# Pixel-Talk/CanonSwap

Hardware: AMD Instinct MI355X
Metric: frames/sec at 512x512 (generator hot path F->W->T->R->W->G) (higher is better)
Workload: dtype f16; 1 GPU; BASELINE configs[2]: 512x512 video, 64 frames batched per launch on each GPU, steady state over 1280 frames (20 launches per GPU) (256x256 crops in, random-init weights of the real architecture); frames_per_launch_per_gpu=64, frames_total=1280, parallelism=frame-shard x1, identities_resident=1, latency_mode=False, accumulate=fp32, debug_decodes=False

## Files before the change

canonswap_amd/_isa.py:

```python
from __future__ import annotations

import os
import subprocess

from ._build import HALO_NGROUPS, OBJ_DIR


def _disassemble(obj_dir: str, objdump: str, oname: str) -> str:
    obj = os.path.join(obj_dir, oname)
    subprocess.run([objdump, "--offloading", obj], check=True, capture_output=True)
    co = obj + ".0.hipv4-amdgcn-amd-amdhsa--gfx950"
    try:
        return subprocess.run([objdump, "-d", "--no-show-raw-insn", co], check=True, capture_output=True, text=True).stdout
    finally:
        for f in os.listdir(obj_dir):
            if f.startswith(oname + ".0."):
                os.remove(os.path.join(obj_dir, f))


def isa_check(obj_dir: str | None = None) -> dict:
    import re
    obj_dir = obj_dir or OBJ_DIR
    objdump = os.environ.get("LLVM_OBJDUMP", "/opt/rocm/lib/llvm/bin/llvm-objdump")
    if not os.path.exists(objdump):
        raise FileNotFoundError(f"isa_check: {objdump} not found")
    seen = dict(_isa_check_wide(obj_dir, objdump))
    seen.update(_isa_check_lat(obj_dir, objdump))
    for g in range(HALO_NGROUPS):
        txt = _disassemble(obj_dir, objdump, f"conv_halo_g{g}.o")
        for m in re.finditer(r"^[0-9a-f]+ <(_Z16conv_halo_kernelILi\d+ELi\d+ELi(\d+)ELi\d+ELi\d+ELi\d+ELb[01]ELb[01]ELi0EEv10ConvParams)>:\n(.*?)(?=^[0-9a-f]+ <|\Z)",
                             txt, re.S | re.M):
            name, wch, body = m.group(1), int(m.group(2)), m.group(3).split("\n")
            want = f"s_waitcnt vmcnt({3 * wch})"
            kend = max(i for i, l in enumerate(body) if "v_mfma" in l)
            waits = [i for i, l in enumerate(body) if i < kend and l.strip().startswith(want) and "lgkmcnt" not in l]
            if len(waits) < 4:
                raise RuntimeError(f"isa_check: {name}: {len(waits)} x `{want}` in the K loop, expected 4 (one per ring slot)")
            waits = waits[:4]
            loads = [(i, re.search(r"global_load_dwordx4 v\[(\d+):(\d+)\], v\[\d+:\d+\], off", l)) for i, l in enumerate(body)]
            loads = [(i, int(q.group(1))) for i, q in loads if q]
            prime = [r for i, r in loads if i < waits[0]][-4 * wch:]
            if len(prime) != 4 * wch:
                raise RuntimeError(f"isa_check: {name}: the prologue primes {len(prime)} ring registers, expected {4 * wch}")
            for k, w in enumerate(waits):
                slot = prime[k * wch:(k + 1) * wch]
                end = waits[k + 1] if k + 1 < 4 else len(body)
                seg = body[w:end]
                rel = [i for i, r in loads if w < i < end and r in slot]
                if len(rel) < wch:
                    raise RuntimeError(f"isa_check: {name}: ring slot {k} is not reloaded into v{slot} after its wait")
                first_reload = min(rel) - w
                uses = [j for j, l in enumerate(seg[:first_reload]) if "v_mfma" in l and any(f"v[{r}:{r + 3}]" in l for r in slot)]
                if not uses:
                    raise RuntimeError(f"isa_check: {name}: no MFMA reads ring slot {k} (v{slot}) between its wait and its reload")
            tail = "\n".join(body[waits[-1]:])
            if "s_waitcnt vmcnt(0)" not in tail:
                raise RuntimeError(f"isa_check: {name}: the ring is not drained (s_waitcnt vmcnt(0)) before the epilogue")
            seen[name] = len(waits)
    if not seen:
        raise RuntimeError("isa_check: no dynamic-shape conv_halo kernel found in the objects (name mangling changed?)")
    return seen


def _isa_check_lat(obj_dir: str, objdump: str) -> dict:
    import re
    txt = _disassemble(obj_dir, objdump, "conv_lat.o")
    seen = {}
    for m in re.finditer(r"^[0-9a-f]+ <(\S*conv_lat_kernel\S*)>:\n(.*?)(?=^[0-9a-f]+ <|\Z)", txt, re.S | re.M):
        name, body = m.group(1), [l.split("//")[0].strip() for l in m.group(2).split("\n")]
        body = [l for l in body if l]
        mf = [i for i, l in enumerate(body) if l.startswith("v_mfma")]
        if not mf:
            raise RuntimeError(f"isa_check: {name}: no MFMA")
        if any(l.startswith(("s_cbranch", "s_branch")) for l in body[mf[0]:mf[-1]]):
            raise RuntimeError(f"isa_check: {name}: a branch inside the K loop (the walk assumes straight-line code)")
        for i, l in enumerate(body):
            if re.search(r"\bm0\b", l):
                ok = l.startswith("s_mov_b32 m0,") and any(b.startswith("buffer_load") and b.endswith("lds") for b in body[i + 1:i + 3])
                if not ok:
                    raise RuntimeError(f"isa_check: {name}: `{l}` touches m0 outside the hidden LDS-DMA sequence")
        nvm, open_dma, nbar, ndma = 0, [], 0, 0
        for i, l in enumerate(body[:mf[-1] + 1]):
            op = l.split()[0]
            if op.startswith(("global_load", "buffer_load", "global_store", "buffer_store", "scratch_load", "scratch_store")):
                if op.startswith("buffer_load") and l.endswith("lds"):
                    open_dma.append(nvm); ndma += 1
                nvm += 1
            if op == "s_barrier":
                nbar += 1
                w = next((body[j] for j in range(i - 1, max(i - 6, -1), -1) if body[j].startswith("s_waitcnt") and "vmcnt" in body[j]), None)
                if w is None and not open_dma:
                    continue
                if w is None:
                    raise RuntimeError(f"isa_check: {name}: barrier {nbar} of the K loop has no vmcnt wait in front of it")
                n = int(re.search(r"vmcnt\((\d+)\)", w).group(1))
                for idx in open_dma:
                    if nvm - idx - 1 < n:
                        raise RuntimeError(f"isa_check: {name}: `{w}` before barrier {nbar} does not cover a DMA piece issued {nvm - idx - 1} vector-memory instructions earlier")
                open_dma = []
        if open_dma:
            raise RuntimeError(f"isa_check: {name}: {len(open_dma)} DMA pieces are never waited for at a chunk head")
        if len(mf) not in (8 * 6 * 8, 8 * 6 * 16) or ndma != 24:
            raise RuntimeError(f"isa_check: {name}: {len(mf)} MFMAs / {ndma} DMA instructions, expected 384 or 768 / 24")
        seen[name] = len(mf)
    if not seen:
        raise RuntimeError("isa_check: no conv_lat kernel found in conv_lat.o (name mangling changed?)")
    return seen


def _isa_check_wide(obj_dir: str, objdump: str) -> dict:
    seen = _isa_check_ring(obj_dir, objdump, "conv_wide.o", r"\S*conv_wide_kernel\S*", 18 * 64)
    seen.update(_isa_check_ring(obj_dir, objdump, "conv_halo_g1.o", r"_Z16conv_halo_kernelILi32ELi8ELi5ELi2ELi2ELi0ELb1ELb0ELi[789]E\S*", None))
    return seen


def _isa_check_ring(obj_dir: str, objdump: str, oname: str, name_re: str, expect_mfma) -> dict:
    import re
    txt = _disassemble(obj_dir, objdump, oname)
    seen = {}
    for m in re.finditer(r"^[0-9a-f]+ <(" + name_re + r")>:\n(.*?)(?=^[0-9a-f]+ <|\Z)", txt, re.S | re.M):
        name, body = m.group(1), m.group(2).split("\n")
        writer, waited, issued, nmfma = {}, {}, {}, 0
        pending, nvm = [], 0
        mf = [i for i, l in enumerate(body) if "v_mfma" in l]
        lo, hi = (mf[0], mf[-1]) if mf else (0, 0)
        for li, l in enumerate(body):
            t = l.split("//")[0].strip()
            if not t:
                continue
            op = t.split()[0]
            if op.startswith("s_waitcnt") and "vmcnt" in t:
                n = int(re.search(r"vmcnt\((\d+)\)", t).group(1))
                for r in waited:
                    if nvm - issued.get(r, -1) - 1 >= n:
                        waited[r] = True
                pending = [q for q in pending if nvm - q[1] - 1 < n]
            if op.startswith(("s_cbranch", "s_branch", "s_endpgm")) or li < lo:
                pending = []
            if pending and not op.startswith(("s_", "global_store", "buffer_store", "ds_write", "scratch_store")):
                mm0 = re.match(r"\S+\s+(v\[(\d+):(\d+)\]|v(\d+))", t)
                if mm0 and not (op.startswith("buffer_load") and t.endswith("lds")):
                    dst = set(range(int(mm0.group(2)), int(mm0.group(3)) + 1)) if mm0.group(2) else {int(mm0.group(4))}
                    for regs, _ in pending:
                        if regs & dst:
                            raise RuntimeError(f"isa_check: {name}: `{t}` writes v{sorted(regs & dst)} while an untracked ring load into them is in flight")
            if op.startswith(("global_load", "buffer_load", "global_store", "buffer_store", "scratch_load", "scratch_store", "global_atomic")):
                if op.startswith("global_load_dwordx4") and li >= lo:
                    q = re.match(r"\S+\s+v\[(\d+):(\d+)\]", t)
                    if q:
                        pending.append((set(range(int(q.group(1)), int(q.group(2)) + 1)), nvm))
                nvm += 1
            if op.startswith("v_mfma"):
                ops = re.findall(r"([av])\[(\d+):(\d+)\]", t)
                if len(ops) < 4 or ops[1][0] != "v":
                    raise RuntimeError(f"isa_check: {name}: MFMA with a weight operand outside the VGPRs: {t}")
                nmfma += 1
                for r in range(int(ops[1][1]), int(ops[1][2]) + 1):
                    if not writer.get(r, "").startswith("global_load_dwordx4"):
                        raise RuntimeError(f"isa_check: {name}: v{r}, a weight operand of `{t}`, was last written by `{writer.get(r)}` (a copy of a ring register?)")
                    if not waited.get(r, False):
                        raise RuntimeError(f"isa_check: {name}: no vmcnt wait between the ring load of v{r} and `{t}`")
                continue
            if op.startswith(("global_store", "buffer_store", "ds_write", "scratch_store", "s_", "buffer_load_dwordx4")) and "lds" in t + " lds" and not op.startswith("global_load"):
                if not op.startswith(("v_", "ds_read", "global_load", "scratch_load")):
                    continue
            mm = re.match(r"\S+\s+(v\[(\d+):(\d+)\]|v(\d+))", t)
            if mm and not op.startswith(("global_store", "buffer_store", "ds_write", "scratch_store")) and not (op.startswith("buffer_load") and t.endswith("lds")):
                rng = range(int(mm.group(2)), int(mm.group(3)) + 1) if mm.group(2) else [int(mm.group(4))]
                is_vm = op.startswith(("global_load", "buffer_load", "scratch_load"))
                for r in rng:
                    writer[r] = op
                    waited[r] = False
                    issued[r] = (nvm - 1) if is_vm else -1
        if expect_mfma is not None and nmfma != expect_mfma:
            raise RuntimeError(f"isa_check: {name}: {nmfma} MFMAs in the kernel, expected {expect_mfma}")
        seen[name] = nmfma
    if not seen:
        raise RuntimeError(f"isa_check: no kernel matching {name_re} found in {oname} (name mangling changed?)")
    return seen
```

canonswap_amd/csrc/vol32.hip:

```cpp
#include "conv_epilogue.h"

namespace {

constexpr int V_TW = 8;
constexpr int V_NC = V_TW + 2;
constexpr int V_CS = 17 * 16;
constexpr int V_RS = V_NC * V_CS;
constexpr int V_WLO = 27 * 2 * 1024;
constexpr int V_SROWS = 8;
enum { V_EPI_F16 = 0,
       V_EPI_RES = 1,
       V_EPI_STAT = 2 };

template <bool SPLIT, int EPI = 0> struct VRing {
    static constexpr int K = SPLIT ? 2 : 4;
    static constexpr int RING = K + 2;
    static constexpr int QS = ((RING * V_RS + 16 + 255) / 256) * 256;
    static constexpr int IMG = 4 * QS;
    static constexpr int NIMG = SPLIT ? 2 : 1;
    static constexpr int AUX = NIMG * IMG;
    static constexpr int RROWS = K + 1;
    static constexpr int RSLOT = 4 * 4096;
    static constexpr int lds(int epi) { return AUX + (SPLIT ? V_WLO : 0) + (epi == 1 ? RROWS * RSLOT : 0); }
};

struct Vol32Params {
    const half_t* in; const half_t* zero;
    int in_sN, in_sH, in_sW;
    int N, H, W;
    const half_t* wgt;
    const float* bias;
    float sl0, sl1;
    const float* res; int res_sN, res_sH, res_sW;
    void* out0; int o0_sN, o0_sH, o0_sW;
    half_t* out1; int o1_sN, o1_sH, o1_sW;
    const float* s2; const float* t2;
    float* stat_out; int stat_nblk;
    int srows;
    const float* xf_y; int xy_sN, xy_sH, xy_sW;
    const float* xf_res; int xr_sN, xr_sH, xr_sW;
    float* xf_out; int xo_sN, xo_sH, xo_sW;
    const float* xf_stats; const float* xf_gamma; const float* xf_beta; float xf_slope;
    int nstrips, nseg, seg_rows, items;
#ifdef V32_TL
    unsigned long long* tl; long tl_cap;
#endif
};

typedef unsigned int u4v __attribute__((ext_vector_type(4)));

#ifdef V32_TL
#define TLS(i) do { __builtin_amdgcn_sched_barrier(0); const unsigned long long t_ = __builtin_amdgcn_s_memtime(); tl_acc[i] += t_ - tl_last; tl_last = t_; \
                    __builtin_amdgcn_sched_barrier(0); } while (0)
#else
#define TLS(i) do { } while (0)
#endif

template <int N> __device__ __forceinline__ void wait_vm() { asm volatile("s_waitcnt vmcnt(%0)" ::"n"(N) : "memory"); }

template <int EPI, bool SPLIT, int XF>
__global__ void __launch_bounds__(256, 1) vol32_kernel(const Vol32Params p)
{
    static_assert(XF == 0 || (SPLIT && EPI == V_EPI_STAT), "transform staging exists for the split-precision statistics kernel");
    extern __shared__ __attribute__((aligned(16))) unsigned char smem[];
    using R = VRing<SPLIT, EPI>;
    constexpr int K = R::K, RING = R::RING, QS = R::QS, IMG = R::IMG, NIMG = R::NIMG;
    constexpr int VOX = SPLIT ? 64 : 32;
    static_assert(!(SPLIT && EPI == V_EPI_RES), "the residual ring and the W_lo fragments share the LDS region after the images");
    constexpr int ND = XF ? 0 : 3 * NIMG + (EPI == V_EPI_RES ? 4 : 0), NR = 0, NS = EPI == V_EPI_F16 ? 2 : (EPI == V_EPI_RES ? 6 : 4);
    constexpr int NW0 = NR + (K - 2) * (ND + NR + NS), NW = NW0 + NS;
    static_assert(NW <= 63, "vmcnt is a 6-bit counter");
    const int tid = threadIdx.x, lane = tid & 63;
    const int wave = __builtin_amdgcn_readfirstlane(tid >> 6);
    const int l15 = lane & 15, l4 = lane >> 4;
#ifdef V32_TL
    unsigned long long tl_acc[10] = {0, 0, 0, 0, 0, 0, 0, 0, 0, 0}, tl_last = __builtin_amdgcn_s_memtime();
#endif

    for (int i = tid * 16; i < NIMG * IMG; i += 256 * 16) *(u4v*)(smem + i) = (u4v){0u, 0u, 0u, 0u};
    h8_t wr[27][2];
    {
        const half_t* wl = p.wgt + ep_lane_row(1, l15) * 32 + l4 * 8;
#pragma unroll
        for (int t = 0; t < 27; ++t) {
            wr[t][0] = *(const h8_t*)(wl + t * 1024 + ep_frag_row(1, 0) * 32);
            wr[t][1] = *(const h8_t*)(wl + t * 1024 + ep_frag_row(1, 1) * 32);
        }
        if constexpr (SPLIT) {
            for (int f = wave; f < 54; f += 4) {
                const h8_t v = *(const h8_t*)(wl + (27 + (f >> 1)) * 1024 + ep_frag_row(1, f & 1) * 32);
                *(h8_t*)(smem + R::AUX + f * 1024 + lane * 16) = v;
            }
        }
    }
    float bias_v[8], s2_v[8], t2_v[8];
#pragma unroll
    for (int r = 0; r < 8; ++r) {
        bias_v[r] = p.bias ? p.bias[l4 * 8 + r] : 0.f;
        s2_v[r] = p.s2 ? p.s2[l4 * 8 + r] : 1.f;
        t2_v[r] = p.s2 ? p.t2[l4 * 8 + r] : 0.f;
    }
    __syncthreads();

    int s_off[3]; bool s_on[3];
#pragma unroll
    for (int j = 0; j < 3; ++j) {
        const int idx = j * 64 + lane, col = idx / 17, ds = idx % 17;
        s_on[j] = idx < V_NC * 17 && ds != 0;
        s_off[j] = col * p.in_sW + (ds - 1) * VOX + wave * 8;
    }
    const int lanebase = l4 * QS + l15 * 16 + (2 * wave) * V_CS;
    const unsigned lane_el = (unsigned)(l15 * 32 + l4 * 8);
    const unsigned char* wlo = smem + R::AUX + lane * 16;

    const int G = (int)gridDim.x;
    int u = (int)blockIdx.x;
    if ((G & 7) == 0) u = (u & 7) * (G >> 3) + (u >> 3);

    for (int item = u; item < p.items; item += G) {
        int t = item;
        const int strip = t % p.nstrips; t /= p.nstrips;
        const int seg = t % p.nseg;
        const int n = t / p.nseg;
        const int w0 = strip * V_TW;
        const int h0 = seg * p.seg_rows, h1 = (h0 + p.seg_rows < p.H) ? h0 + p.seg_rows : p.H;
        bool c_ok[3];
#pragma unroll
        for (int j = 0; j < 3; ++j) {
            const int col = (j * 64 + lane) / 17;
            c_ok[j] = s_on[j] && (unsigned)(w0 - 1 + col) < (unsigned)p.W;
        }
        const half_t* in_n = p.in + (long)n * p.in_sN + (long)(w0 - 1) * p.in_sW;
        const unsigned nb_o0 = (unsigned)(n * p.o0_sN + (w0 + 2 * wave) * p.o0_sW);
        const unsigned nb_o1 = (unsigned)(n * p.o1_sN + (w0 + 2 * wave) * p.o1_sW);
        const unsigned nb_rs = (unsigned)(n * p.res_sN + (w0 + 2 * wave) * p.res_sW);
        auto stage_piece = [&](int r, int slot, int rslot, int q) {
            if (q < 3 * NIMG) {
                const int im = q / 3, j = q % 3;
                const bool rok = (unsigned)r < (unsigned)p.H && r <= h1;
                const half_t* rp = in_n + (long)r * p.in_sH;
                unsigned char* dst = smem + wave * QS + slot * V_RS;
                if (s_on[j]) {
                    const half_t* src = (rok && c_ok[j]) ? rp + s_off[j] + im * 32 : p.zero;
                    __builtin_amdgcn_global_load_lds((const __attribute__((address_space(1))) void*)src,
                                                     (__attribute__((address_space(3))) void*)(dst + im * IMG + j * 1024), 16, 0, 0);
                }
            } else if constexpr (EPI == V_EPI_RES) {
                const int j = q - 3 * NIMG;
                const int rc = (unsigned)r < (unsigned)p.H ? r : 0;
                const float* rsrc = p.res + (nb_rs + (unsigned)(rc * p.res_sH) + lane_el);
                unsigned char* rdst = smem + R::AUX + rslot * R::RSLOT + wave * 4096;
                __builtin_amdgcn_global_load_lds((const __attribute__((address_space(1))) void*)(rsrc + (j >> 1) * p.res_sW + (j & 1) * 4),
                                                 (__attribute__((address_space(3))) void*)(rdst + j * 1024), 16, 0, 0);
            }
        };
        auto stage_row = [&](int r, int slot, int rslot) {
#pragma unroll
            for (int q = 0; q < ND; ++q) stage_piece(r, slot, rslot, q);
        };
        constexpr bool XRES = XF >= 2 && ((XF - 2) & 1) != 0, XWB = XF >= 2 && ((XF - 2) & 2) != 0;
        float4 xr[XF ? 3 : 1][2], xs[XRES ? 3 : 1][2];
        float xsc[XF >= 2 ? 8 : 1], xsh[XF >= 2 ? 8 : 1];
        const int xq = tid & 3;
        if constexpr (XF >= 2) {
#pragma unroll
            for (int r = 0; r < 8; ++r) {
                const int c = xq * 8 + r;
                const float mean = p.xf_stats[((long)n * 32 + c) * 2], rstd = p.xf_stats[((long)n * 32 + c) * 2 + 1];
                xsc[r] = gn_scale(rstd, p.xf_gamma[c]);
                xsh[r] = gn_shift(mean, xsc[r], p.xf_beta[c]);
            }
        }
        int xoff[XF ? 3 : 1]; bool xcok[XF ? 3 : 1];
        if constexpr (XF != 0) {
#pragma unroll
            for (int it = 0; it < 3; ++it) {
                int idx = it * 256 + tid;
                if (idx >= V_NC * 64) idx -= 128;
                const int col = idx >> 6, d = (idx >> 2) & 15;
                xoff[it] = n * p.xy_sN + (w0 - 1 + col) * p.xy_sW + d * 32 + xq * 8;
                xcok[it] = (unsigned)(w0 - 1 + col) < (unsigned)p.W;
            }
        }
        const unsigned xsafe = (unsigned)(n * p.xy_sN + w0 * p.xy_sW + h0 * p.xy_sH + ((tid >> 2) & 15) * 32 + xq * 8);
        auto xf_load_to = [&](int r, int it, float4 (&dr)[2], float4 (&ds)[2]) {
            if constexpr (XF != 0) {
                const bool okl = xcok[it] && (unsigned)r < (unsigned)p.H && r <= h1;
                const unsigned o = okl ? (unsigned)(xoff[it] + r * p.xy_sH) : xsafe;
                const float* y = p.xf_y + o;
                dr[0] = *(const float4*)y; dr[1] = *(const float4*)(y + 4);
                if constexpr (XRES) {
                    const float* x = p.xf_res + o;
                    ds[0] = *(const float4*)x; ds[1] = *(const float4*)(x + 4);
                }
            }
        };
        auto xf_load = [&](int r, int it) { xf_load_to(r, it, xr[it], xs[XRES ? it : 0]); };
        float xa[8];
        auto xf_write_from = [&](int r, int slot, int it, int part, const float4 (&xr)[2], const float4 (&xs)[2]) {
            if constexpr (XF != 0) {
                int idx = it * 256 + tid;
                if (idx >= V_NC * 64) idx -= 128;
                const bool ok = xcok[it] && (unsigned)r < (unsigned)p.H && r <= h1;
#pragma unroll
                for (int k = 0; k < 8; ++k) {
                    if (part >= 0 && (k >> 2) != part) continue;
                    const float v = ((const float*)&xr[k >> 2])[k & 3];
                    if constexpr (XRES) xa[k] = gn_lrelu(v, xsc[k], xsh[k], ((const float*)&xs[k >> 2])[k & 3], p.xf_slope);
                    else if constexpr (XF >= 2) xa[k] = gn_lrelu(v, xsc[k], xsh[k], 0.f, p.xf_slope);
                    else xa[k] = v;
                    if (!ok) xa[k] = 0.f;
                }
                if (part >= 0 && part != 2) return;
                h8_t hi, lo;
#pragma unroll
                for (int k = 0; k < 8; ++k) { hi[k] = (half_t)xa[k]; lo[k] = (half_t)(xa[k] - (float)hi[k]); }
                unsigned char* dst = smem + xq * QS + (idx >> 6) * V_CS + (((idx >> 2) & 15) + 1) * 16 + slot * V_RS;
                *(h8_t*)dst = hi; *(h8_t*)(dst + IMG) = lo;
                if constexpr (XWB) {
                    float* o = ok ? p.xf_out + (unsigned)(xoff[it] + r * p.xy_sH) : (float*)p.zero;
                    *(float4*)o = make_float4(xa[0], xa[1], xa[2], xa[3]); *(float4*)(o + 4) = make_float4(xa[4], xa[5], xa[6], xa[7]);
                }
            }
        };
        auto xf_write = [&](int r, int slot, int it, int part) { xf_write_from(r, slot, it, part, xr[it], xs[XRES ? it : 0]); };
        if constexpr (XF != 0) {
            float4 pr[3][3][2], ps[XRES ? 3 : 1][3][2];
#pragma unroll
            for (int i = 0; i < 3; ++i)
#pragma unroll
                for (int it = 0; it < 3; ++it) xf_load_to(h0 - 1 + i, it, pr[i][it], ps[XRES ? i : 0][it]);
#pragma unroll
            for (int i = 0; i < 3; ++i)
#pragma unroll
                for (int it = 0; it < 3; ++it) xf_write_from(h0 - 1 + i, i, it, -1, pr[i][it], ps[XRES ? i : 0][it]);
        } else {
#pragma unroll
            for (int i = 0; i <= K; ++i) stage_row(h0 - 1 + i, i, i == 0 ? K : i - 1);
        }
        TLS(0);
        __syncthreads();
        TLS(1);

        float ov[2][8]; h8_t ou[2];
        bool have = false;
        int hprev = 0;
        auto store_piece = [&](int k) {
            constexpr int PC = NS / 2;
            const int c = k / PC, w = k % PC;
            const unsigned o = nb_o0 + (unsigned)(hprev * p.o0_sH + c * p.o0_sW) + lane_el;
            if constexpr (EPI != V_EPI_F16) {
                if (w == 0) *(float4*)((float*)p.out0 + o) = make_float4(ov[c][0], ov[c][1], ov[c][2], ov[c][3]);
                if (w == 1) *(float4*)((float*)p.out0 + o + 4) = make_float4(ov[c][4], ov[c][5], ov[c][6], ov[c][7]);
                if constexpr (EPI == V_EPI_RES) {
                    if (w == 2) *(h8_t*)(p.out1 + (nb_o1 + (unsigned)(hprev * p.o1_sH + c * p.o1_sW) + lane_el)) = ou[c];
                }
            } else {
                h8_t x;
#pragma unroll
                for (int r = 0; r < 8; ++r) x[r] = ep_h(ov[c][r]);
                *(h8_t*)((half_t*)p.out0 + o) = x;
            }
        };
        auto flush = [&]() {
#pragma unroll
            for (int k = 0; k < NS; ++k) store_piece(k);
        };
        float st_s[8], st_q[8];
#pragma unroll
        for (int r = 0; r < 8; ++r) { st_s[r] = 0.f; st_q[r] = 0.f; }

        int s0 = 0, r0 = 0;
        for (int h = h0; h < h1; ++h) {
            int sk = s0 + K + 1; sk -= sk >= RING ? RING : 0;
            int rk = r0 + K; rk -= rk >= R::RROWS ? R::RROWS : 0;
            f4_t rr[2][2];
            if constexpr (EPI == V_EPI_RES) {
#pragma unroll
                for (int c = 0; c < 2; ++c)
#pragma unroll
                    for (int i = 0; i < 2; ++i) rr[c][i] = *(const f4_t*)(wlo + r0 * R::RSLOT + wave * 4096 + (c * 2 + i) * 1024);
            }
            int rb[3];
#pragma unroll
            for (int kh = 0; kh < 3; ++kh) { int sl = s0 + kh; sl -= sl >= RING ? RING : 0; rb[kh] = lanebase + sl * V_RS; }
            f4_t acc[2][2];
#pragma unroll
            for (int c = 0; c < 2; ++c)
#pragma unroll
                for (int ci = 0; ci < 2; ++ci) acc[c][ci] = (f4_t){0.f, 0.f, 0.f, 0.f};
            constexpr int NG = SPLIT ? 27 : 9;
            constexpr int XL0 = 4, XW0 = 17;
            h8_t fa[4], fb[4];
            h8_t wa[SPLIT ? 3 : 1][2], wb[SPLIT ? 3 : 1][2];
            auto rd = [&](h8_t (&f)[4], h8_t (&wl2)[SPLIT ? 3 : 1][2], int G2) {
                const int pass = G2 / 9, g = G2 % 9, kd = g / 3, kh = g % 3;
                const int img = (SPLIT && pass == 2) ? IMG : 0;
#pragma unroll
                for (int i = 0; i < 4; ++i) f[i] = *(const h8_t*)(smem + rb[kh] + img + i * V_CS + kd * 16);
                if constexpr (SPLIT) {
                    if (pass == 1) {
#pragma unroll
                        for (int kw = 0; kw < 3; ++kw)
#pragma unroll
                            for (int ci = 0; ci < 2; ++ci) wl2[kw][ci] = *(const h8_t*)(wlo + ((g * 3 + kw) * 2 + ci) * 1024);
                    }
                }
            };
            rd(fa, wa, 0);
#pragma unroll
            for (int G2 = 0; G2 < NG; ++G2) {
                h8_t (&cur)[4] = (G2 & 1) ? fb : fa;
                h8_t (&wcur)[SPLIT ? 3 : 1][2] = (G2 & 1) ? wb : wa;
                h8_t (&wnxt)[SPLIT ? 3 : 1][2] = (G2 & 1) ? wa : wb;
                if constexpr (XF != 0) { if (G2 >= XW0 && G2 < XW0 + 9) xf_write(h + 2, sk, (G2 - XW0) / 3, (G2 - XW0) % 3); }
                if (G2 + 1 < NG) {
                    h8_t (&nxt)[4] = (G2 & 1) ? fa : fb;
                    rd(nxt, wnxt, G2 + 1);
                }
                const int pass = G2 / 9, g = G2 % 9;
#pragma unroll
                for (int kw = 0; kw < 3; ++kw)
#pragma unroll
                    for (int c = 0; c < 2; ++c)
#pragma unroll
                        for (int ci = 0; ci < 2; ++ci) {
                            const h8_t a = (SPLIT && pass == 1) ? wcur[SPLIT ? kw : 0][ci] : wr[g * 3 + kw][ci];
                            acc[c][ci] = __builtin_amdgcn_mfma_f32_16x16x32_f16(a, cur[kw + c], acc[c][ci], 0, 0, 0);
                        }
                if (G2 + 1 < NG) {
                    const int nrd = 4 + ((SPLIT && (G2 + 1) / 9 == 1) ? 6 : 0);
                    const bool conv_here = XF != 0 && G2 >= XW0 && G2 < XW0 + 9;
#pragma unroll
                    for (int i = 0; i < 11; ++i) {
                        __builtin_amdgcn_sched_group_barrier(0x008, 1, 0);
                        if (i < nrd) __builtin_amdgcn_sched_group_barrier(0x100, 1, 0);
                        if (conv_here) __builtin_amdgcn_sched_group_barrier(0x002, 4, 0);
                    }
                }
                __builtin_amdgcn_sched_barrier(0);
                if constexpr (XF == 0) {
                    constexpr int NM = ND + NS;
#pragma unroll
                    for (int m = G2 * NM / NG; m < (G2 + 1) * NM / NG; ++m) {
                        asm volatile("" ::: "memory");
                        if (m < ND) stage_piece(h + K, sk, rk, m);
                        else if (have) store_piece(m - ND);
                        asm volatile("" ::: "memory");
                    }
                    __builtin_amdgcn_sched_barrier(0);
                } else {
                    if (G2 < NS && have) store_piece(G2);
                    if (G2 >= XL0 && G2 < XL0 + 6 && ((G2 - XL0) & 1) == 0) xf_load(h + 2, (G2 - XL0) >> 1);
                    __builtin_amdgcn_sched_barrier(0);
                }
            }
            TLS(4);
#pragma unroll
            for (int c = 0; c < 2; ++c) {
#pragma unroll
                for (int r = 0; r < 8; ++r) {
                    float v = acc[c][r >> 2][r & 3] + bias_v[r];
                    v = lin_act(v, p.sl0);
                    if constexpr (EPI == V_EPI_RES) v += rr[c][r >> 2][r & 3];
                    ov[c][r] = v;
                    if constexpr (EPI == V_EPI_STAT) { st_s[r] += v; st_q[r] = fmaf(v, v, st_q[r]); }
                    if constexpr (EPI == V_EPI_RES) {
                        const float a = v * s2_v[r] + t2_v[r];
                        ou[c][r] = ep_h(lin_act(a, p.sl1));
                    }
                }
            }
            if constexpr (EPI == V_EPI_STAT) {
                if (((h + 1) % p.srows) == 0 || h + 1 == h1) {
                    const int blk = (h / p.srows) * (p.W / 2) + (w0 / 2 + wave);
                    float pa[8], pb[8];
#pragma unroll
                    for (int r = 0; r < 8; ++r) {
                        float a = st_s[r], b = st_q[r];
                        st_s[r] = 0.f; st_q[r] = 0.f;
#pragma unroll
                        for (int o = 1; o < 16; o <<= 1) { a += __shfl_xor(a, o, 64); b += __shfl_xor(b, o, 64); }
                        pa[r] = a; pb[r] = b;
                    }
                    if (l15 == 0) {
                        float4* dst = (float4*)(p.stat_out + (((long)n * p.stat_nblk + blk) * 32 + l4 * 8) * 2);
#pragma unroll
                        for (int r = 0; r < 4; ++r) dst[r] = make_float4(pa[2 * r], pb[2 * r], pa[2 * r + 1], pb[2 * r + 1]);
                    }
                }
            }
            have = true; hprev = h;
            s0 = s0 + 1 == RING ? 0 : s0 + 1;
            r0 = r0 + 1 == R::RROWS ? 0 : r0 + 1;
            TLS(5);
            if constexpr (XF != 0) asm volatile("s_waitcnt lgkmcnt(0)" ::: "memory");
            else if (h > h0 + K - 2) wait_vm<NW>();
            else wait_vm<NW0>();
            TLS(6);
            __builtin_amdgcn_s_barrier();
            asm volatile("" ::: "memory");
            TLS(7);
#ifdef V32_TL
            tl_acc[9] += 1;
#endif
        }
        if (have) flush();
        __syncthreads();
        TLS(8);
    }
#ifdef V32_TL
    if (p.tl && lane == 0) {
        const long wi = (long)blockIdx.x * 4 + wave;
        if (wi < p.tl_cap) {
            unsigned hwid;
            asm volatile("s_getreg_b32 %0, hwreg(HW_REG_HW_ID)" : "=s"(hwid));
            unsigned long long* o = p.tl + wi * 12;
#pragma unroll
            for (int i = 0; i < 10; ++i) o[i] = tl_acc[i];
            o[10] = hwid; o[11] = __builtin_amdgcn_s_memrealtime();
        }
    }
#endif
}

int g_ncu = 0;
#ifdef V32_TL
unsigned long long* g_v32_tl = nullptr;
long g_v32_cap = 0;
#endif

}

#ifdef V32_TL
extern "C" void cs_debug_set_vol32_tl(void* buf, long cap) { g_v32_tl = (unsigned long long*)buf; g_v32_cap = cap; }
#endif

bool vol32_supported(const ConvParams& p)
{
    if (p.KD != 3 || p.KH != 3 || p.KW != 3 || p.Cout_pad != 32 || p.Cout != 32 || p.D != 16 || p.inD != 16 || (p.W % V_TW) != 0) return false;
    if (p.xf_kind) {
        if (!p.hilo || p.Cin != 96 || !p.stat_out || (p.xf_kind != 1 && p.xf_kind != 2) || !p.xf_y.p || p.xf_y.sD != 32) return false;
        if (p.xf_kind == 2 && (!p.xf_stats || !p.xf_gamma || !p.xf_beta)) return false;
        if (p.xf_res.p && (p.xf_kind != 2 || p.xf_res.sD != 32)) return false;
        if (p.xf_out.p && (p.xf_kind != 2 || p.xf_out.sD != 32)) return false;
    } else if (p.hilo ? (p.Cin != 96 || p.in_sD != 64) : (p.Cin != 32 || p.in_sD != 32)) return false;
    if (p.up_shift || p.cg || p.wslot || p.sk_out || p.ragged || p.pixscale || p.stats || p.pool_hw || p.spmul) return false;
    if (p.act0 > ACT_LRELU || p.act1 > ACT_LRELU) return false;
    if (p.res.p && (!p.res_f32 || p.res.sD != 32)) return false;
    if (p.out0.p && p.out0.sD != 32) return false;
    if (p.out1.p && p.out1.sD != 32) return false;
    if (!p.out0.p) return false;
    if (p.hilo && !p.stat_out) return false;
    if (p.stat_out) return p.out0_f32 && !p.res.p && !p.out1.p;
    if (p.res.p) return p.out0_f32 && p.out1.p && !p.hilo;
    return !p.out0_f32 && !p.out1.p;
}

static int vol32_srows(const ConvParams& p) { return p.v32_srows > 0 ? p.v32_srows : V_SROWS; }
int vol32_stat_nblk(const ConvParams& p) { const int sr = vol32_srows(p); return ((p.H + sr - 1) / sr) * (p.W / 2); }

int launch_vol32(const ConvParams& p, hipStream_t st)
{
    if (!vol32_supported(p)) { cs_set_error("vol32: not a 3x3x3 32 -> 32 convolution on a [N][H][W][16][32] volume this kernel supports"); return -1; }
    if (ep_check_extents(p, "vol32")) return -1;
    const long in_span = (long)(p.N - 1) * p.in_sN + (long)(p.H - 1) * p.in_sH + (long)(p.W - 1) * p.in_sW + 1024;
    if (!p.xf_kind && in_span >= (1L << 31)) { cs_set_error("vol32: the input spans 2^31 elements or more"); return -1; }
    if (!g_ncu) {
        int dev = 0, n = 0;
        if (hipGetDevice(&dev) != hipSuccess || hipDeviceGetAttribute(&n, hipDeviceAttributeMultiprocessorCount, dev) != hipSuccess || n < 1) n = 256;
        g_ncu = n;
    }
    Vol32Params k;
    k.in = p.in; k.zero = p.zero; k.in_sN = (int)p.in_sN; k.in_sH = (int)p.in_sH; k.in_sW = (int)p.in_sW;
    k.N = p.N; k.H = p.H; k.W = p.W;
    k.wgt = p.wgt; k.bias = p.bias;
    k.sl0 = p.act0 == ACT_NONE ? 1.f : (p.act0 == ACT_LRELU ? p.slope0 : 0.f);
    k.sl1 = p.act1 == ACT_NONE ? 1.f : (p.act1 == ACT_LRELU ? p.slope1 : 0.f);
    k.res = (const float*)p.res.p; k.res_sN = (int)p.res.sN; k.res_sH = (int)p.res.sH; k.res_sW = (int)p.res.sW;
    k.out0 = p.out0.p; k.o0_sN = (int)p.out0.sN; k.o0_sH = (int)p.out0.sH; k.o0_sW = (int)p.out0.sW;
    k.out1 = (half_t*)p.out1.p; k.o1_sN = (int)p.out1.sN; k.o1_sH = (int)p.out1.sH; k.o1_sW = (int)p.out1.sW;
    k.s2 = p.s2; k.t2 = p.t2;
    k.stat_out = p.stat_out; k.stat_nblk = vol32_stat_nblk(p); k.srows = vol32_srows(p);
    k.xf_y = (const float*)p.xf_y.p; k.xy_sN = (int)p.xf_y.sN; k.xy_sH = (int)p.xf_y.sH; k.xy_sW = (int)p.xf_y.sW;
    k.xf_res = (const float*)p.xf_res.p; k.xr_sN = (int)p.xf_res.sN; k.xr_sH = (int)p.xf_res.sH; k.xr_sW = (int)p.xf_res.sW;
    k.xf_out = (float*)p.xf_out.p; k.xo_sN = (int)p.xf_out.sN; k.xo_sH = (int)p.xf_out.sH; k.xo_sW = (int)p.xf_out.sW;
    k.xf_stats = p.xf_stats; k.xf_gamma = p.xf_gamma; k.xf_beta = p.xf_beta; k.xf_slope = p.xf_slope;
    if (p.xf_kind) {
        auto same = [&](const TDesc& t) { return !t.p || (t.sN == p.xf_y.sN && t.sH == p.xf_y.sH && t.sW == p.xf_y.sW); };
        if (!same(p.xf_res) || !same(p.xf_out)) { cs_set_error("vol32: the transform-staging volumes must share their strides"); return -1; }
        const long lim = 1L << 31;
        auto span = [&](const TDesc& t) { return (long)(p.N - 1) * t.sN + (long)(p.H - 1) * t.sH + (long)(p.W - 1) * t.sW + 512; };
        if (span(p.xf_y) >= lim || (p.xf_res.p && span(p.xf_res) >= lim) || (p.xf_out.p && span(p.xf_out) >= lim)) {
            cs_set_error("vol32: a transform-staging tensor spans 2^31 elements or more"); return -1;
        }
    }
#ifdef V32_TL
    k.tl = g_v32_tl; k.tl_cap = g_v32_cap;
#endif
    k.nstrips = p.W / V_TW;
    int nseg = 1;
    while ((long)p.N * k.nstrips * nseg < g_ncu && (p.H % (nseg * 2 * k.srows)) == 0) nseg *= 2;
    k.seg_rows = (p.H + nseg - 1) / nseg;
    k.nseg = (p.H + k.seg_rows - 1) / k.seg_rows;
    k.items = p.N * k.nstrips * k.nseg;
    int grid = k.items < g_ncu ? k.items : g_ncu;
    if (grid >= 8) grid &= ~7;
    const bool split = p.hilo != 0;
    const int epi = p.stat_out ? V_EPI_STAT : (p.res.p ? V_EPI_RES : V_EPI_F16);
    auto go = [&](auto kern, size_t lds) -> int {
        if (lds > 64 * 1024) {
            hipError_t e = hipFuncSetAttribute((const void*)kern, hipFuncAttributeMaxDynamicSharedMemorySize, (int)lds);
            if (e != hipSuccess) { cs_set_error("vol32: opting into %zu bytes of LDS failed: %s", lds, hipGetErrorString(e)); return -1; }
        }
        hipLaunchKernelGGL(kern, dim3((unsigned)grid), dim3(256), lds, st, k);
        return 0;
    };
    int r = -1;
    if (split) {
        if (epi != V_EPI_STAT) { cs_set_error("vol32: the split-precision kernel exists with the statistics epilogue only"); return -1; }
        if (p.xf_kind == 2) {
            const int v = (p.xf_res.p ? 1 : 0) | (p.xf_out.p ? 2 : 0);
            if (v == 0) r = go(vol32_kernel<V_EPI_STAT, true, 2>, VRing<true, V_EPI_STAT>::lds(V_EPI_STAT));
            else if (v == 1) r = go(vol32_kernel<V_EPI_STAT, true, 3>, VRing<true, V_EPI_STAT>::lds(V_EPI_STAT));
            else if (v == 2) r = go(vol32_kernel<V_EPI_STAT, true, 4>, VRing<true, V_EPI_STAT>::lds(V_EPI_STAT));
            else r = go(vol32_kernel<V_EPI_STAT, true, 5>, VRing<true, V_EPI_STAT>::lds(V_EPI_STAT));
        }
        else if (p.xf_kind == 1) r = go(vol32_kernel<V_EPI_STAT, true, 1>, VRing<true, V_EPI_STAT>::lds(V_EPI_STAT));
        else r = go(vol32_kernel<V_EPI_STAT, true, 0>, VRing<true, V_EPI_STAT>::lds(V_EPI_STAT));
    } else {
        if (epi == V_EPI_STAT) r = go(vol32_kernel<V_EPI_STAT, false, 0>, VRing<false, V_EPI_STAT>::lds(V_EPI_STAT));
        else if (epi == V_EPI_RES) r = go(vol32_kernel<V_EPI_RES, false, 0>, VRing<false, V_EPI_RES>::lds(V_EPI_RES));
        else r = go(vol32_kernel<V_EPI_F16, false, 0>, VRing<false, V_EPI_F16>::lds(V_EPI_F16));
    }
    if (r) return r;
    hipError_t e = hipGetLastError();
    if (e != hipSuccess) { cs_set_error("vol32 launch: %s", hipGetErrorString(e)); return -1; }
    return 0;
}
```

Baseline: 545.2 frames/s.

## Pin vol32 weights in AGPRs, make stores branchless, spread transform conversion

Result: no change. 546.6 frames/s, median of 6 (+0.3%).

```diff
diff --git a/canonswap_amd/_isa.py b/canonswap_amd/_isa.py
--- a/canonswap_amd/_isa.py
+++ b/canonswap_amd/_isa.py
@@ -6,12 +6,16 @@
 from ._build import HALO_NGROUPS, OBJ_DIR
 
 
-def _disassemble(obj_dir: str, objdump: str, oname: str) -> str:
+def _disassemble(obj_dir: str, objdump: str, oname: str, notes: bool = False):
     obj = os.path.join(obj_dir, oname)
     subprocess.run([objdump, "--offloading", obj], check=True, capture_output=True)
     co = obj + ".0.hipv4-amdgcn-amd-amdhsa--gfx950"
     try:
-        return subprocess.run([objdump, "-d", "--no-show-raw-insn", co], check=True, capture_output=True, text=True).stdout
+        txt = subprocess.run([objdump, "-d", "--no-show-raw-insn", co], check=True, capture_output=True, text=True).stdout
+        if not notes:
+            return txt
+        readelf = os.path.join(os.path.dirname(objdump), "llvm-readelf")
+        return txt, subprocess.run([readelf, "--notes", co], check=True, capture_output=True, text=True).stdout
     finally:
         for f in os.listdir(obj_dir):
             if f.startswith(oname + ".0."):
@@ -26,6 +30,7 @@
         raise FileNotFoundError(f"isa_check: {objdump} not found")
     seen = dict(_isa_check_wide(obj_dir, objdump))
     seen.update(_isa_check_lat(obj_dir, objdump))
+    seen.update(_isa_check_vol32(obj_dir, objdump))
     for g in range(HALO_NGROUPS):
         txt = _disassemble(obj_dir, objdump, f"conv_halo_g{g}.o")
         for m in re.finditer(r"^[0-9a-f]+ <(_Z16conv_halo_kernelILi\d+ELi\d+ELi(\d+)ELi\d+ELi\d+ELi\d+ELb[01]ELb[01]ELi0EEv10ConvParams)>:\n(.*?)(?=^[0-9a-f]+ <|\Z)",
@@ -108,6 +113,73 @@
     return seen
 
 
+VOL32_STEP_MFMAS = {True: 324, False: 108}
+VOL32_COPY_BOUND = 8
+
+
+def vol32_kernel_meta(notes: str) -> dict:
+    import re
+    meta = {}
+    for blk in re.split(r"\n\s+- (?=\.agpr_count:)", notes):
+        name = re.search(r"\.name:\s+(\S+)", blk)
+        keys = {k: re.search(r"\." + key + r":\s+(\d+)", blk) for k, key in (("agpr", "agpr_count"), ("vgpr", "vgpr_count"), ("private", "private_segment_fixed_size"))}
+        if name and all(keys.values()):
+            meta[name.group(1)] = {k: int(v.group(1)) for k, v in keys.items()}
+    return meta
+
+
+def vol32_check_kernel(name: str, body: list, meta: dict) -> int:
+    import re
+    k = re.search(r"vol32_kernelILi(\d+)ELb([01])ELi(\d+)E", name)
+    if not k:
+        raise RuntimeError(f"isa_check: {name}: not a vol32_kernel instantiation")
+    split, xf = k.group(2) == "1", int(k.group(3))
+    if meta.get("private", -1) != 0:
+        raise RuntimeError(f"isa_check: {name}: private segment of {meta.get('private')} bytes (scratch), expected 0")
+    if not 0 < meta.get("vgpr", 0) <= 512 or meta.get("agpr", 0) > 256:
+        raise RuntimeError(f"isa_check: {name}: {meta.get('vgpr')} registers in total, {meta.get('agpr')} AGPRs: over the 512 / 256 of one wave per SIMD")
+    body = [l.split("//")[0].strip() for l in body]
+    body = [l for l in body if l]
+    mf = [i for i, l in enumerate(body) if l.startswith("v_mfma")]
+    per = VOL32_STEP_MFMAS[split]
+    if not mf or len(mf) % per:
+        raise RuntimeError(f"isa_check: {name}: {len(mf)} MFMAs, expected whole steps of {per}")
+    nskip = (6 if split else 3) if xf == 0 else 0
+    for s in range(len(mf) // per):
+        lo, hi = mf[s * per], mf[(s + 1) * per - 1]
+        step = body[lo:hi + 1]
+        copies = sum(1 for l in step if l.startswith("v_accvgpr_"))
+        if copies > VOL32_COPY_BOUND:
+            raise RuntimeError(f"isa_check: {name}: {copies} AGPR <-> VGPR copies inside a step, at most {VOL32_COPY_BOUND} expected (weights not held in AGPRs by declaration?)")
+        skips = 0
+        for i, l in enumerate(step):
+            if not l.startswith(("s_cbranch", "s_branch", "s_setpc", "s_call")):
+                continue
+            q = re.match(r"s_cbranch_execz\s+(\d+)", l)
+            if q and any(x.startswith("global_load_lds") for x in step[i + 1:i + 1 + int(q.group(1))]):
+                skips += 1
+                continue
+            raise RuntimeError(f"isa_check: {name}: `{l}` between the MFMAs of a step")
+        if skips > nskip:
+            raise RuntimeError(f"isa_check: {name}: {skips} exec-mask skips of DMA pieces inside a step, at most {nskip} expected")
+    return len(mf) // per
+
+
+def _isa_check_vol32(obj_dir: str, objdump: str) -> dict:
+    import re
+    txt, notes = _disassemble(obj_dir, objdump, "vol32.o", notes=True)
+    meta = vol32_kernel_meta(notes)
+    seen = {}
+    for m in re.finditer(r"^[0-9a-f]+ <(\S*vol32_kernelILi\S*)>:\n(.*?)(?=^[0-9a-f]+ <|\Z)", txt, re.S | re.M):
+        name = m.group(1)
+        if name not in meta:
+            raise RuntimeError(f"isa_check: {name}: no metadata record in the code object's notes")
+        seen[name] = vol32_check_kernel(name, m.group(2).split("\n"), meta[name])
+    if len(seen) < 9:
+        raise RuntimeError(f"isa_check: {len(seen)} vol32_kernel instantiations found in vol32.o, expected 9 (name mangling changed?)")
+    return seen
+
+
 def _isa_check_wide(obj_dir: str, objdump: str) -> dict:
     seen = _isa_check_ring(obj_dir, objdump, "conv_wide.o", r"\S*conv_wide_kernel\S*", 18 * 64)
     seen.update(_isa_check_ring(obj_dir, objdump, "conv_halo_g1.o", r"_Z16conv_halo_kernelILi32ELi8ELi5ELi2ELi2ELi0ELb1ELb0ELi[789]E\S*", None))
diff --git a/canonswap_amd/csrc/vol32.hip b/canonswap_amd/csrc/vol32.hip
--- a/canonswap_amd/csrc/vol32.hip
+++ b/canonswap_amd/csrc/vol32.hip
@@ -49,6 +49,13 @@
 
 typedef unsigned int u4v __attribute__((ext_vector_type(4)));
 
+constexpr unsigned V_ALL_TAPS = (1u << 27) - 1;
+constexpr unsigned v32_agpr_taps(int EPI, bool SPLIT, int XF)
+{
+    (void)EPI; (void)SPLIT; (void)XF;
+    return V_ALL_TAPS;
+}
+
 #ifdef V32_TL
 #define TLS(i) do { __builtin_amdgcn_sched_barrier(0); const unsigned long long t_ = __builtin_amdgcn_s_memtime(); tl_acc[i] += t_ - tl_last; tl_last = t_; \
                     __builtin_amdgcn_sched_barrier(0); } while (0)
@@ -68,7 +75,7 @@
     constexpr int VOX = SPLIT ? 64 : 32;
     static_assert(!(SPLIT && EPI == V_EPI_RES), "the residual ring and the W_lo fragments share the LDS region after the images");
     constexpr int ND = XF ? 0 : 3 * NIMG + (EPI == V_EPI_RES ? 4 : 0), NR = 0, NS = EPI == V_EPI_F16 ? 2 : (EPI == V_EPI_RES ? 6 : 4);
-    constexpr int NW0 = NR + (K - 2) * (ND + NR + NS), NW = NW0 + NS;
+    constexpr int NW = NR + NS + (K - 2) * (ND + NR + NS);
     static_assert(NW <= 63, "vmcnt is a 6-bit counter");
     const int tid = threadIdx.x, lane = tid & 63;
     const int wave = __builtin_amdgcn_readfirstlane(tid >> 6);
@@ -85,6 +92,10 @@
         for (int t = 0; t < 27; ++t) {
             wr[t][0] = *(const h8_t*)(wl + t * 1024 + ep_frag_row(1, 0) * 32);
             wr[t][1] = *(const h8_t*)(wl + t * 1024 + ep_frag_row(1, 1) * 32);
+        }
+#pragma unroll
+        for (int t = 0; t < 27; ++t) {
+            if ((v32_agpr_taps(EPI, SPLIT, XF) >> t) & 1) { asm volatile("" : "+a"(wr[t][0])); asm volatile("" : "+a"(wr[t][1])); }
         }
         if constexpr (SPLIT) {
             for (int f = wave; f < 54; f += 4) {
@@ -197,6 +208,7 @@
         };
         auto xf_load = [&](int r, int it) { xf_load_to(r, it, xr[it], xs[XRES ? it : 0]); };
         float xa[8];
+        h8_t xhi, xlo;
         auto xf_write_from = [&](int r, int slot, int it, int part, const float4 (&xr)[2], const float4 (&xs)[2]) {
             if constexpr (XF != 0) {
                 int idx = it * 256 + tid;
@@ -211,12 +223,14 @@
                     else xa[k] = v;
                     if (!ok) xa[k] = 0.f;
                 }
-                if (part >= 0 && part != 2) return;
-                h8_t hi, lo;
-#pragma unroll
-                for (int k = 0; k < 8; ++k) { hi[k] = (half_t)xa[k]; lo[k] = (half_t)(xa[k] - (float)hi[k]); }
+#pragma unroll
+                for (int k = 0; k < 8; ++k) {
+                    if (part >= 0 && 2 + (k >> 2) != part) continue;
+                    xhi[k] = (half_t)xa[k]; xlo[k] = (half_t)(xa[k] - (float)xhi[k]);
+                }
+                if (part >= 0 && part != 3) return;
                 unsigned char* dst = smem + xq * QS + (idx >> 6) * V_CS + (((idx >> 2) & 15) + 1) * 16 + slot * V_RS;
-                *(h8_t*)dst = hi; *(h8_t*)(dst + IMG) = lo;
+                *(h8_t*)dst = xhi; *(h8_t*)(dst + IMG) = xlo;
                 if constexpr (XWB) {
                     float* o = ok ? p.xf_out + (unsigned)(xoff[it] + r * p.xy_sH) : (float*)p.zero;
                     *(float4*)o = make_float4(xa[0], xa[1], xa[2], xa[3]); *(float4*)(o + 4) = make_float4(xa[4], xa[5], xa[6], xa[7]);
@@ -243,23 +257,31 @@
         TLS(1);
 
         float ov[2][8]; h8_t ou[2];
+#pragma unroll
+        for (int c = 0; c < 2; ++c) {
+#pragma unroll
+            for (int r = 0; r < 8; ++r) { ov[c][r] = 0.f; ou[c][r] = (half_t)0.f; }
+        }
         bool have = false;
         int hprev = 0;
         auto store_piece = [&](int k) {
             constexpr int PC = NS / 2;
             const int c = k / PC, w = k % PC;
-            const unsigned o = nb_o0 + (unsigned)(hprev * p.o0_sH + c * p.o0_sW) + lane_el;
+            const unsigned o = have ? nb_o0 + (unsigned)(hprev * p.o0_sH + c * p.o0_sW) + lane_el : 0u;
             if constexpr (EPI != V_EPI_F16) {
-                if (w == 0) *(float4*)((float*)p.out0 + o) = make_float4(ov[c][0], ov[c][1], ov[c][2], ov[c][3]);
-                if (w == 1) *(float4*)((float*)p.out0 + o + 4) = make_float4(ov[c][4], ov[c][5], ov[c][6], ov[c][7]);
+                float* d0 = have ? (float*)p.out0 : (float*)p.zero;
+                if (w == 0) *(float4*)(d0 + o) = make_float4(ov[c][0], ov[c][1], ov[c][2], ov[c][3]);
+                if (w == 1) *(float4*)(d0 + o + 4) = make_float4(ov[c][4], ov[c][5], ov[c][6], ov[c][7]);
                 if constexpr (EPI == V_EPI_RES) {
-                    if (w == 2) *(h8_t*)(p.out1 + (nb_o1 + (unsigned)(hprev * p.o1_sH + c * p.o1_sW) + lane_el)) = ou[c];
+                    half_t* d1 = have ? p.out1 + (nb_o1 + (unsigned)(hprev * p.o1_sH + c * p.o1_sW) + lane_el) : (half_t*)p.zero;
+                    if (w == 2) *(h8_t*)d1 = ou[c];
                 }
             } else {
                 h8_t x;
 #pragma unroll
                 for (int r = 0; r < 8; ++r) x[r] = ep_h(ov[c][r]);
-                *(h8_t*)((half_t*)p.out0 + o) = x;
+                half_t* d0 = have ? (half_t*)p.out0 : (half_t*)p.zero;
+                *(h8_t*)(d0 + o) = x;
             }
         };
         auto flush = [&]() {
@@ -290,7 +312,7 @@
 #pragma unroll
                 for (int ci = 0; ci < 2; ++ci) acc[c][ci] = (f4_t){0.f, 0.f, 0.f, 0.f};
             constexpr int NG = SPLIT ? 27 : 9;
-            constexpr int XL0 = 4, XW0 = 17;
+            constexpr int XL0 = 2, XW0 = 15;
             h8_t fa[4], fb[4];
             h8_t wa[SPLIT ? 3 : 1][2], wb[SPLIT ? 3 : 1][2];
             auto rd = [&](h8_t (&f)[4], h8_t (&wl2)[SPLIT ? 3 : 1][2], int G2) {
@@ -313,7 +335,7 @@
                 h8_t (&cur)[4] = (G2 & 1) ? fb : fa;
                 h8_t (&wcur)[SPLIT ? 3 : 1][2] = (G2 & 1) ? wb : wa;
                 h8_t (&wnxt)[SPLIT ? 3 : 1][2] = (G2 & 1) ? wa : wb;
-                if constexpr (XF != 0) { if (G2 >= XW0 && G2 < XW0 + 9) xf_write(h + 2, sk, (G2 - XW0) / 3, (G2 - XW0) % 3); }
+                if constexpr (XF != 0) { if (G2 >= XW0 && G2 < XW0 + 12) xf_write(h + 2, sk, (G2 - XW0) / 4, (G2 - XW0) % 4); }
                 if (G2 + 1 < NG) {
                     h8_t (&nxt)[4] = (G2 & 1) ? fa : fb;
                     rd(nxt, wnxt, G2 + 1);
@@ -328,14 +350,15 @@
                             const h8_t a = (SPLIT && pass == 1) ? wcur[SPLIT ? kw : 0][ci] : wr[g * 3 + kw][ci];
                             acc[c][ci] = __builtin_amdgcn_mfma_f32_16x16x32_f16(a, cur[kw + c], acc[c][ci], 0, 0, 0);
                         }
-                if (G2 + 1 < NG) {
-                    const int nrd = 4 + ((SPLIT && (G2 + 1) / 9 == 1) ? 6 : 0);
-                    const bool conv_here = XF != 0 && G2 >= XW0 && G2 < XW0 + 9;
+                const bool conv_here = XF != 0 && G2 >= XW0 && G2 < XW0 + 12;
+                if (G2 + 1 < NG || conv_here) {
+                    const int nrd = G2 + 1 < NG ? 4 + ((SPLIT && (G2 + 1) / 9 == 1) ? 6 : 0) : 0;
 #pragma unroll
                     for (int i = 0; i < 11; ++i) {
                         __builtin_amdgcn_sched_group_barrier(0x008, 1, 0);
                         if (i < nrd) __builtin_amdgcn_sched_group_barrier(0x100, 1, 0);
-                        if (conv_here) __builtin_amdgcn_sched_group_barrier(0x002, 4, 0);
+                        if (conv_here && i < nrd) __builtin_amdgcn_sched_group_barrier(0x002, 1, 0);
+                        if (conv_here && i >= nrd) __builtin_amdgcn_sched_group_barrier(0x002, 2, 0);
                     }
                 }
                 __builtin_amdgcn_sched_barrier(0);
@@ -345,12 +368,12 @@
                     for (int m = G2 * NM / NG; m < (G2 + 1) * NM / NG; ++m) {
                         asm volatile("" ::: "memory");
                         if (m < ND) stage_piece(h + K, sk, rk, m);
-                        else if (have) store_piece(m - ND);
+                        else store_piece(m - ND);
                         asm volatile("" ::: "memory");
                     }
                     __builtin_amdgcn_sched_barrier(0);
                 } else {
-                    if (G2 < NS && have) store_piece(G2);
+                    if (G2 < NS) store_piece(G2);
                     if (G2 >= XL0 && G2 < XL0 + 6 && ((G2 - XL0) & 1) == 0) xf_load(h + 2, (G2 - XL0) >> 1);
                     __builtin_amdgcn_sched_barrier(0);
                 }
@@ -395,8 +418,7 @@
             r0 = r0 + 1 == R::RROWS ? 0 : r0 + 1;
             TLS(5);
             if constexpr (XF != 0) asm volatile("s_waitcnt lgkmcnt(0)" ::: "memory");
-            else if (h > h0 + K - 2) wait_vm<NW>();
-            else wait_vm<NW0>();
+            else wait_vm<NW>();
             TLS(6);
             __builtin_amdgcn_s_barrier();
             asm volatile("" ::: "memory");
```
